# yumingj/Text2Human

Measured on AMD Instinct MI355X. Metric: 512x256 images/sec (sample_from_parsing), higher is better.
Workload: dtype f16 hi plane + e4m3 cross-term planes, f32 accumulate (hidden err 4e-5, tokens exact); exact-f32: exact_fp32_path

## Files before the change

### text2human_amd/csrc/attention.hip

```cpp
#include <stdlib.h>

#include <type_traits>

#include "common.h"

namespace {

constexpr int HD = 64;
constexpr int QB = 128;
constexpr int KT = 64;
constexpr int K_LD = 68;
constexpr int V_LD = 64;
constexpr int O_LD = 68;
constexpr int KV_TILE = KT * K_LD + KT * V_LD;

__global__ __launch_bounds__(512) void mha_kernel(const float* __restrict__ qkv,
                                                  float* __restrict__ y, int T, int C,
                                                  int n_head, uint16_t* __restrict__ y_split, int* ovf) {
  __shared__ __attribute__((aligned(16))) float smem[2 * KV_TILE];
  static_assert(2 * KV_TILE >= 4 * 32 * 64 + 4 * 32 * O_LD, "LDS reuse layout");

  const int tid = threadIdx.x, lane = tid & 63, wave = tid >> 6;
  const int l31 = lane & 31, hh = lane >> 5;
  const int qw = wave & 3, kh = wave >> 2;
  int qt, head, b;
  {
    const int nqt = T / QB, total = gridDim.x, id = blockIdx.x;
    const int xcd = id & 7, slot = id >> 3, q = total >> 3, r = total & 7;
    const int lin = (xcd < r ? xcd * (q + 1) : r * (q + 1) + (xcd - r) * q) + slot;
    qt = lin % nqt;
    const int hb = lin / nqt;
    head = hb % n_head;
    b = hb / n_head;
  }
  const int q0 = qt * QB + qw * 32;
  const int ld = 3 * C;
  const float* base = qkv + (int64_t)b * T * ld + head * HD;

  float qf[32];
  {
    const float* qp = base + (int64_t)(q0 + l31) * ld + 32 * hh;
#pragma unroll
    for (int s4 = 0; s4 < 8; ++s4) {
      const f32x4 v = *reinterpret_cast<const f32x4*>(qp + 4 * s4);
#pragma unroll
      for (int e = 0; e < 4; ++e) qf[4 * s4 + e] = v[e] * 0.125f;
    }
  }

  f32x16 o_acc[2];
#pragma unroll
  for (int dt = 0; dt < 2; ++dt)
#pragma unroll
    for (int r = 0; r < 16; ++r) o_acc[dt][r] = 0.f;
  float m_run = -INFINITY, l_run = 0.f;

  const int s_half = tid >> 8, s_t = tid & 255;
  const int s_col4 = s_t & 15, s_row0 = s_t >> 4;
  float* const Ks_st = smem + s_half * KV_TILE;
  float* const Vs_st = Ks_st + KT * K_LD;
  const int half_keys = T / 2;
  f32x4 kreg[4], vreg[4];
  auto load_kv = [&](int it) {
#pragma unroll
    for (int i = 0; i < 4; ++i) {
      const int key = s_half * half_keys + it * KT + s_row0 + 16 * i;
      const float* p = base + (int64_t)key * ld + s_col4 * 4;
      kreg[i] = *reinterpret_cast<const f32x4*>(p + C);
      vreg[i] = *reinterpret_cast<const f32x4*>(p + 2 * C);
    }
  };
  auto store_kv = [&]() {
#pragma unroll
    for (int i = 0; i < 4; ++i) {
      const int r = s_row0 + 16 * i;
      *reinterpret_cast<f32x4*>(Ks_st + r * K_LD + s_col4 * 4) = kreg[i];
      *reinterpret_cast<f32x4*>(Vs_st + r * V_LD + s_col4 * 4) = vreg[i];
    }
  };

  const float* const Ks = smem + kh * KV_TILE;
  const float* const Vs = Ks + KT * K_LD;
  const int nit = half_keys / KT;
  load_kv(0);
  for (int it = 0; it < nit; ++it) {
    __syncthreads();
    store_kv();
    __syncthreads();
    if (it + 1 < nit) load_kv(it + 1);

#pragma unroll
    for (int ks = 0; ks < 2; ++ks) {
      f32x16 st;
#pragma unroll
      for (int r = 0; r < 16; ++r) st[r] = 0.f;
      const float* kp = Ks + (ks * 32 + l31) * K_LD + 32 * hh;
#pragma unroll
      for (int j = 0; j < 8; ++j) {
        const f32x4 kf = *reinterpret_cast<const f32x4*>(kp + 4 * j);
#pragma unroll
        for (int e = 0; e < 4; ++e)
          st = __builtin_amdgcn_mfma_f32_32x32x2f32(kf[e], qf[4 * j + e], st, 0, 0, 0);
      }
      float mx = st[0];
#pragma unroll
      for (int r = 1; r < 16; ++r) mx = fmaxf(mx, st[r]);
      mx = fmaxf(mx, __shfl_xor(mx, 32, 64));
      const float m_new = fmaxf(m_run, mx);
      const float alpha = (m_run == -INFINITY) ? 0.f : fast_exp(m_run - m_new);
      float psum = 0.f;
#pragma unroll
      for (int r = 0; r < 16; ++r) {
        st[r] = fast_exp(st[r] - m_new);
        psum += st[r];
      }
      psum += __shfl_xor(psum, 32, 64);
      l_run = l_run * alpha + psum;
      m_run = m_new;
#pragma unroll
      for (int dt = 0; dt < 2; ++dt)
#pragma unroll
        for (int r = 0; r < 16; ++r) o_acc[dt][r] *= alpha;
#pragma unroll
      for (int s = 0; s < 16; ++s) {
        const int key = ks * 32 + (s & 3) + 8 * (s >> 2) + 4 * hh;
        const float* vp = Vs + key * V_LD + l31;
#pragma unroll
        for (int dt = 0; dt < 2; ++dt)
          o_acc[dt] = __builtin_amdgcn_mfma_f32_32x32x2f32(vp[32 * dt], st[s], o_acc[dt], 0, 0, 0);
      }
    }
  }

  __syncthreads();
  float* const Ox = smem;
  float* const Mx = smem + 4 * 32 * 64;
  float* const Lx = Mx + 4 * 64;
  if (kh == 1) {
#pragma unroll
    for (int dt = 0; dt < 2; ++dt)
#pragma unroll
      for (int r = 0; r < 16; ++r) Ox[(qw * 32 + dt * 16 + r) * 64 + lane] = o_acc[dt][r];
    Mx[qw * 64 + lane] = m_run;
    Lx[qw * 64 + lane] = l_run;
  }
  __syncthreads();
  float inv_l = 0.f;
  if (kh == 0) {
    const float m2 = Mx[qw * 64 + lane], l2 = Lx[qw * 64 + lane];
    const float m = fmaxf(m_run, m2);
    const float a1 = expf(m_run - m), a2 = expf(m2 - m);
#pragma unroll
    for (int dt = 0; dt < 2; ++dt)
#pragma unroll
      for (int r = 0; r < 16; ++r)
        o_acc[dt][r] = o_acc[dt][r] * a1 + Ox[(qw * 32 + dt * 16 + r) * 64 + lane] * a2;
    inv_l = 1.0f / (l_run * a1 + l2 * a2);
  }
  __syncthreads();
  float* Os = smem + 4 * 32 * 64 + qw * 32 * O_LD;
  if (kh == 0) {
#pragma unroll
    for (int dt = 0; dt < 2; ++dt)
#pragma unroll
      for (int r = 0; r < 16; ++r) {
        const int d = dt * 32 + (r & 3) + 8 * (r >> 2) + 4 * hh;
        Os[l31 * O_LD + d] = o_acc[dt][r] * inv_l;
      }
  }
  __syncthreads();
  if (kh == 0) {
    const int64_t grow = (int64_t)b * T + q0;
#pragma unroll
    for (int it = 0; it < 4; ++it) {
      const int row = it * 8 + (lane >> 3), c8 = (lane & 7) * 8;
      const f32x4 va = *reinterpret_cast<const f32x4*>(Os + row * O_LD + c8);
      const f32x4 vb = *reinterpret_cast<const f32x4*>(Os + row * O_LD + c8 + 4);
      if (y) {
        *reinterpret_cast<f32x4*>(y + (grow + row) * C + head * HD + c8) = va;
        *reinterpret_cast<f32x4*>(y + (grow + row) * C + head * HD + c8 + 4) = vb;
      }
      if (y_split) t2h_store_split8(y_split, grow + row, C, head * HD + c8, va, vb, ovf);
    }
  }
}


typedef t2h_f16x8 f16x8;
typedef unsigned int u32x4 __attribute__((ext_vector_type(4)));

template <int J>
__device__ __forceinline__ void split8(const f32x16& x, f16x8& hi, f16x8& lo) {
#pragma unroll
  for (int e = 0; e < 8; ++e) {
    _Float16 a, b;
    t2h_split2(x[8 * J + e], a, b);
    hi[e] = a;
    lo[e] = b;
  }
}

#ifndef T2H_MHA_PACKED
#define T2H_MHA_PACKED 0
#endif
#ifdef T2H_MHA_TIMING
__device__ long long* g_mha_timing = nullptr;
#define TM_NOW() clock64()
#else
#define TM_NOW() 0ll
#endif

__device__ __forceinline__ void half_barrier(int* ctr, int target, int lane) {
  asm volatile("s_waitcnt lgkmcnt(0)" ::: "memory");
  if (lane == 0) __hip_atomic_fetch_add(ctr, 1, __ATOMIC_RELAXED, __HIP_MEMORY_SCOPE_WORKGROUP);
  while (__hip_atomic_load(ctr, __ATOMIC_RELAXED, __HIP_MEMORY_SCOPE_WORKGROUP) < target) __builtin_amdgcn_s_sleep(1);
  asm volatile("" ::: "memory");
}

constexpr int DK_TILE = KT * 256;
constexpr int DV_TILE = 2 * HD * 128;
constexpr int DKV_TILE = DK_TILE + DV_TILE;

template <int KH>
__global__ __launch_bounds__(512) void mha_split_pipe_kernel(const uint16_t* __restrict__ qk, int ld_cols,
                                                        const uint16_t* __restrict__ vt, float* __restrict__ y,
                                                        uint16_t* __restrict__ y_split, int T, int C, int n_head,
                                                        int* ovf, float y_x8_scale) {
  constexpr int NQW = 8 / KH;
  constexpr int EPI_B = KH == 2 ? (4 * 32 * 64 + 4 * 32 * O_LD) * 4 : NQW * 32 * O_LD * 4;
  constexpr int SMEM_B = 2 * KH * DKV_TILE > EPI_B ? 2 * KH * DKV_TILE : EPI_B;
  __shared__ __attribute__((aligned(16))) char smem_raw[SMEM_B + 16];
  float* const smem = reinterpret_cast<float*>(smem_raw);
  int* const bar = reinterpret_cast<int*>(smem_raw + SMEM_B);

  const int tid = threadIdx.x, lane = tid & 63;
  const int wave = __builtin_amdgcn_readfirstlane(tid >> 6);
  const long long tm0 = TM_NOW();
#ifdef T2H_MHA_TIMING
  const long long rt0 = (long long)__builtin_amdgcn_s_memrealtime();
#endif
  long long tm_stage = 0, tm_comp = 0;
  if (tid < 2) bar[tid] = 0;
  __syncthreads();
  const int l31 = lane & 31, hh = lane >> 5;
  const int qw = KH == 2 ? (wave & 3) : wave, kh = KH == 2 ? (wave >> 2) : 0;
  int qt, head, b;
  {
    const int nqt = T / (32 * NQW), total = gridDim.x, id = blockIdx.x;
    const int xcd = id & 7, slot = id >> 3, q = total >> 3, r = total & 7;
    const int lin = (xcd < r ? xcd * (q + 1) : r * (q + 1) + (xcd - r) * q) + slot;
    qt = lin % nqt;
    const int hb = lin / nqt;
    head = hb % n_head;
    b = hb / n_head;
  }
  const int q0 = qt * (32 * NQW) + qw * 32;
  const int64_t row_b = (int64_t)(ld_cols / 32) * T2H_SPLIT_TILE_B;
  const char* const qk_b = reinterpret_cast<const char*>(qk) + (int64_t)b * T * row_b;
  const int q_tile0 = 2 * head, k_tile0 = C / 32 + 2 * head;

  f16x8 qf[4][2];
  {
    const char* qp = qk_b + (int64_t)(q0 + l31) * row_b + q_tile0 * T2H_SPLIT_TILE_B + hh * 16;
#pragma unroll
    for (int kk = 0; kk < 4; ++kk)
#pragma unroll
      for (int pl = 0; pl < 2; ++pl)
        qf[kk][pl] = *reinterpret_cast<const f16x8*>(qp + (kk >> 1) * T2H_SPLIT_TILE_B + pl * 64 + (kk & 1) * 32);
  }

  f32x16 o_acc[2], o_lo[2];
#pragma unroll
  for (int dt = 0; dt < 2; ++dt)
#pragma unroll
    for (int r = 0; r < 16; ++r) o_acc[dt][r] = o_lo[dt][r] = 0.f;
  float m_run = -INFINITY, l_run = 0.f;

  const int half_keys = T / KH;
  const int w4 = qw;
  constexpr int CPW = 16 / NQW;
  const char* const vt_b = reinterpret_cast<const char*>(vt) + ((int64_t)(b * n_head + head) * 2 * HD) * T * 2;
  const unsigned lds_half = (unsigned)(uintptr_t)smem_raw + kh * (2 * DKV_TILE);
  const char* const kbase = qk_b + (int64_t)(kh * half_keys) * row_b + k_tile0 * T2H_SPLIT_TILE_B;
  const char* const vbase = vt_b + (int64_t)(kh * half_keys) * 2;
  const unsigned k_rowoff = (unsigned)(4 * CPW * w4 + (lane >> 4)) * (unsigned)row_b;
  const unsigned k_b16 = (unsigned)((lane & 15) ^ (lane >> 4) ^ ((4 * CPW * w4) & 15)) * 16;
  const unsigned v_rowoff = (unsigned)(8 * CPW * w4 + (lane >> 3)) * (unsigned)(T * 2);
  const unsigned v_b16 = (unsigned)((lane & 7) ^ (lane >> 4) ^ ((4 * CPW * w4) & 7)) * 16;
  auto dma16 = [&](unsigned voff, const char* sbase, unsigned lds_dst) {
    unsigned keep;
#ifndef T2H_MHA_DMA_POLICY
#define T2H_MHA_DMA_POLICY ""
#endif
    asm volatile("s_mov_b32 %0, m0\n\ts_mov_b32 m0, %3\n\ts_nop 0\n\tglobal_load_lds_dwordx4 %1, %2" T2H_MHA_DMA_POLICY "\n\ts_mov_b32 m0, %0"
                 : "=&s"(keep)
                 : "v"(voff), "s"(sbase), "s"(lds_dst)
                 : "memory");
  };
  auto dma_k = [&](int it, int buf) {
    const char* const sb = kbase + (int64_t)it * KT * row_b;
    const unsigned dst = __builtin_amdgcn_readfirstlane(lds_half + buf * DKV_TILE + CPW * w4 * 1024);
#pragma unroll
    for (int i = 0; i < CPW; ++i) dma16(k_rowoff + (unsigned)(4 * i) * (unsigned)row_b + (k_b16 ^ (64u * i)), sb, dst + i * 1024);
  };
  auto dma_v = [&](int it, int buf) {
    const char* const sb = vbase + it * KT * 2;
    const unsigned dst = __builtin_amdgcn_readfirstlane(lds_half + buf * DKV_TILE + DK_TILE + CPW * w4 * 1024);
#pragma unroll
    for (int i = 0; i < CPW; ++i) dma16(v_rowoff + (unsigned)(8 * i) * (unsigned)(T * 2) + (v_b16 ^ (64u * (i & 1))), sb, dst + i * 1024);
  };
  auto dma_landed = [] { asm volatile("s_waitcnt vmcnt(0)" ::: "memory"); };

  const char* const Ks0 = smem_raw + kh * (2 * DKV_TILE);
  const int nit = half_keys / KT;
  const unsigned xk16 = (unsigned)(hh ^ (l31 & 15)) * 16, xv16 = (unsigned)(hh ^ ((l31 >> 1) & 7)) * 16;
  auto s_tile = [&](const char* Ks, f32x16 (&st)[2], f32x16 (&st_lo)[2]) {
#pragma unroll
    for (int ks = 0; ks < 2; ++ks)
#pragma unroll
      for (int r = 0; r < 16; ++r) st[ks][r] = st_lo[ks][r] = 0.f;
#pragma unroll
    for (int kk = 0; kk < 4; ++kk) {
      f16x8 kf[2][2];
#pragma unroll
      for (int ks = 0; ks < 2; ++ks)
#pragma unroll
        for (int pl = 0; pl < 2; ++pl)
          kf[ks][pl] = *reinterpret_cast<const f16x8*>(
              Ks + (ks * 32 + l31) * 256 + ((unsigned)(((kk >> 1) * 8 + pl * 4 + (kk & 1) * 2) * 16) ^ xk16));
      st_lo[0] = __builtin_amdgcn_mfma_f32_32x32x16_f16(kf[0][1], qf[kk][0], st_lo[0], 0, 0, 0);
      st_lo[1] = __builtin_amdgcn_mfma_f32_32x32x16_f16(kf[1][1], qf[kk][0], st_lo[1], 0, 0, 0);
      st[0] = __builtin_amdgcn_mfma_f32_32x32x16_f16(kf[0][0], qf[kk][0], st[0], 0, 0, 0);
      st_lo[0] = __builtin_amdgcn_mfma_f32_32x32x16_f16(kf[0][0], qf[kk][1], st_lo[0], 0, 0, 0);
      st_lo[1] = __builtin_amdgcn_mfma_f32_32x32x16_f16(kf[1][0], qf[kk][1], st_lo[1], 0, 0, 0);
      st[1] = __builtin_amdgcn_mfma_f32_32x32x16_f16(kf[1][0], qf[kk][0], st[1], 0, 0, 0);
    }
  };

  int bar_n = 0;
  const long long tm1 = TM_NOW();
#ifdef T2H_MHA_TIMING
  const long long rt1 = (long long)__builtin_amdgcn_s_memrealtime();
#endif
  if (KH == 2 && kh == 1) __builtin_amdgcn_s_setprio(1);
  constexpr float SC = 0.125f * 1.44269504088896340736f;
  f32x16 sc[2];
  {
    f32x16 st[2], st_lo[2];
    dma_k(0, 0);
    dma_v(0, 0);
    if (nit > 1) dma_k(1, 1);
    dma_landed();
    half_barrier(bar + kh, bar_n += NQW, lane);
    s_tile(Ks0, st, st_lo);
#pragma unroll
    for (int ks = 0; ks < 2; ++ks)
#pragma unroll
      for (int r = 0; r < 16; ++r) sc[ks][r] = fmaf(st_lo[ks][r], T2H_SPLIT_LO_INV, st[ks][r]);
    half_barrier(bar + kh, bar_n += NQW, lane);
  }
  auto iteration = [&](int it, auto next_c) {
    constexpr bool NEXT = decltype(next_c)::value;
    const long long tb = TM_NOW();
    const int buf = it & 1;
    const char* const Vs = Ks0 + buf * DKV_TILE + DK_TILE;
    if (it + 2 < nit) dma_k(it + 2, buf);
    if (it + 1 < nit) dma_v(it + 1, buf ^ 1);
    float mx = -INFINITY;
#pragma unroll
    for (int ks = 0; ks < 2; ++ks)
#pragma unroll
      for (int r = 0; r < 16; ++r) mx = fmaxf(mx, sc[ks][r]);
    mx = fmaxf(mx, __shfl_xor(mx, 32, 64)) * SC;
    const float m_new = fmaxf(m_run, mx);
    if (__any(m_new > m_run)) {
      const float alpha = (m_run == -INFINITY) ? 0.f : __builtin_amdgcn_exp2f(m_run - m_new);
      l_run *= alpha;
#pragma unroll
      for (int dt = 0; dt < 2; ++dt)
#pragma unroll
        for (int r = 0; r < 16; ++r) {
          o_acc[dt][r] *= alpha;
          o_lo[dt][r] *= alpha;
        }
      m_run = m_new;
    }
    f32x16 sn[2], sn_lo[2];
    if constexpr (NEXT) s_tile(Ks0 + (buf ^ 1) * DKV_TILE, sn, sn_lo);
    float psum = 0.f;
#if T2H_MHA_PACKED
    typedef float f32x2_ __attribute__((ext_vector_type(2)));
    const f32x2_ sc2 = {SC, SC}, nm2 = {-m_run, -m_run};
    f32x2_ ps2 = {0.f, 0.f};
#endif
#pragma unroll
    for (int ks = 0; ks < 2; ++ks) {
#if T2H_MHA_PACKED
#pragma unroll
      for (int r = 0; r < 16; r += 2) {
        f32x2_ a = {sc[ks][r], sc[ks][r + 1]};
        a = __builtin_elementwise_fma(a, sc2, nm2);
        a[0] = __builtin_amdgcn_exp2f(a[0]);
        a[1] = __builtin_amdgcn_exp2f(a[1]);
        sc[ks][r] = a[0];
        sc[ks][r + 1] = a[1];
        ps2 += a;
      }
#else
#pragma unroll
      for (int r = 0; r < 16; ++r) {
        sc[ks][r] = __builtin_amdgcn_exp2f(fmaf(sc[ks][r], SC, -m_run));
        psum += sc[ks][r];
      }
#endif
#pragma unroll
      for (int j = 0; j < 2; ++j) {
        f16x8 pf[2];
        if (j == 0) split8<0>(sc[ks], pf[0], pf[1]);
        else split8<1>(sc[ks], pf[0], pf[1]);
        f16x8 vf[2][2];
#pragma unroll
        for (int dt = 0; dt < 2; ++dt)
#pragma unroll
          for (int pl = 0; pl < 2; ++pl)
            vf[dt][pl] = *reinterpret_cast<const f16x8*>(Vs + (pl * HD + dt * 32 + l31) * 128 +
                                                          ((unsigned)((ks * 4 + j * 2) * 16) ^ xv16));
        o_lo[0] = __builtin_amdgcn_mfma_f32_32x32x16_f16(vf[0][1], pf[0], o_lo[0], 0, 0, 0);
        o_lo[1] = __builtin_amdgcn_mfma_f32_32x32x16_f16(vf[1][1], pf[0], o_lo[1], 0, 0, 0);
        o_acc[0] = __builtin_amdgcn_mfma_f32_32x32x16_f16(vf[0][0], pf[0], o_acc[0], 0, 0, 0);
        o_lo[0] = __builtin_amdgcn_mfma_f32_32x32x16_f16(vf[0][0], pf[1], o_lo[0], 0, 0, 0);
        o_lo[1] = __builtin_amdgcn_mfma_f32_32x32x16_f16(vf[1][0], pf[1], o_lo[1], 0, 0, 0);
        o_acc[1] = __builtin_amdgcn_mfma_f32_32x32x16_f16(vf[1][0], pf[0], o_acc[1], 0, 0, 0);
      }
    }
#if T2H_MHA_PACKED
    psum = ps2[0] + ps2[1];
#endif
    psum += __shfl_xor(psum, 32, 64);
    l_run += psum;
    if constexpr (NEXT) {
#pragma unroll
      for (int ks = 0; ks < 2; ++ks)
#pragma unroll
        for (int r = 0; r < 16; ++r) sc[ks][r] = fmaf(sn_lo[ks][r], T2H_SPLIT_LO_INV, sn[ks][r]);
    }
    const long long tc = TM_NOW();
    tm_comp += tc - tb;
    if constexpr (NEXT) {
      dma_landed();
      half_barrier(bar + kh, bar_n += NQW, lane);
    }
    tm_stage += TM_NOW() - tc;
  };
  for (int it = 0; it + 1 < nit; ++it) iteration(it, std::true_type{});
  iteration(nit - 1, std::false_type{});

#pragma unroll
  for (int dt = 0; dt < 2; ++dt)
#pragma unroll
    for (int r = 0; r < 16; ++r) o_acc[dt][r] = fmaf(o_lo[dt][r], T2H_SPLIT_LO_INV, o_acc[dt][r]);
  const long long tm2 = TM_NOW();
#ifdef T2H_MHA_TIMING
  const long long rt2 = (long long)__builtin_amdgcn_s_memrealtime();
#endif
  __syncthreads();
  if constexpr (KH == 2) {
  float* const Ox = smem;
  float* const Mx = smem + 4 * 32 * 64;
  float* const Lx = Mx + 4 * 64;
  if (kh == 1) {
#pragma unroll
    for (int dt = 0; dt < 2; ++dt)
#pragma unroll
      for (int r = 0; r < 16; ++r) Ox[(qw * 32 + dt * 16 + r) * 64 + lane] = o_acc[dt][r];
    Mx[qw * 64 + lane] = m_run;
    Lx[qw * 64 + lane] = l_run;
  }
  __syncthreads();
  float inv_l = 0.f;
  if (kh == 0) {
    const float m2 = Mx[qw * 64 + lane], l2 = Lx[qw * 64 + lane];
    const float m = fmaxf(m_run, m2);
    const float a1 = exp2f(m_run - m), a2 = exp2f(m2 - m);
#pragma unroll
    for (int dt = 0; dt < 2; ++dt)
#pragma unroll
      for (int r = 0; r < 16; ++r)
        o_acc[dt][r] = o_acc[dt][r] * a1 + Ox[(qw * 32 + dt * 16 + r) * 64 + lane] * a2;
    inv_l = 1.0f / (l_run * a1 + l2 * a2);
  }
  __syncthreads();
  float* Os = smem + 4 * 32 * 64 + qw * 32 * O_LD;
  if (kh == 0) {
#pragma unroll
    for (int dt = 0; dt < 2; ++dt)
#pragma unroll
      for (int r = 0; r < 16; ++r) {
        const int d = dt * 32 + (r & 3) + 8 * (r >> 2) + 4 * hh;
        Os[l31 * O_LD + d] = o_acc[dt][r] * inv_l;
      }
  }
  __syncthreads();
  {
    const int64_t grow = (int64_t)b * T + q0;
#pragma unroll
    for (int it2 = 0; it2 < 2; ++it2) {
      const int it = it2 + 2 * kh;
      const int row = it * 8 + (lane >> 3), c8 = (lane & 7) * 8;
      const f32x4 va = *reinterpret_cast<const f32x4*>(Os + row * O_LD + c8);
      const f32x4 vb = *reinterpret_cast<const f32x4*>(Os + row * O_LD + c8 + 4);
      if (y) {
        *reinterpret_cast<f32x4*>(y + (grow + row) * C + head * HD + c8) = va;
        *reinterpret_cast<f32x4*>(y + (grow + row) * C + head * HD + c8 + 4) = vb;
      }
      if (y_split) {
        if (y_x8_scale > 0.f) t2h_store_x8_8<1>(y_split, grow + row, C, head * HD + c8, va, vb, y_x8_scale, ovf);
        else t2h_store_split8(y_split, grow + row, C, head * HD + c8, va, vb, ovf);
      }
    }
  }
  } else {
    const float inv_l = 1.0f / l_run;
    float* const Os = smem + qw * 32 * O_LD;
#pragma unroll
    for (int dt = 0; dt < 2; ++dt)
#pragma unroll
      for (int r = 0; r < 16; ++r) {
        const int d = dt * 32 + (r & 3) + 8 * (r >> 2) + 4 * hh;
        Os[l31 * O_LD + d] = o_acc[dt][r] * inv_l;
      }
    asm volatile("s_waitcnt lgkmcnt(0)" ::: "memory");
    const int64_t grow = (int64_t)b * T + q0;
#pragma unroll
    for (int it = 0; it < 4; ++it) {
      const int row = it * 8 + (lane >> 3), c8 = (lane & 7) * 8;
      const f32x4 va = *reinterpret_cast<const f32x4*>(Os + row * O_LD + c8);
      const f32x4 vb = *reinterpret_cast<const f32x4*>(Os + row * O_LD + c8 + 4);
      if (y) {
        *reinterpret_cast<f32x4*>(y + (grow + row) * C + head * HD + c8) = va;
        *reinterpret_cast<f32x4*>(y + (grow + row) * C + head * HD + c8 + 4) = vb;
      }
      if (y_split) {
        if (y_x8_scale > 0.f) t2h_store_x8_8<1>(y_split, grow + row, C, head * HD + c8, va, vb, y_x8_scale, ovf);
        else t2h_store_split8(y_split, grow + row, C, head * HD + c8, va, vb, ovf);
      }
    }
  }
#ifdef T2H_MHA_TIMING
  if (g_mha_timing && blockIdx.x == 8 && lane == 0 && (wave == 0 || wave == 4)) {
    long long* o = g_mha_timing + (wave == 4 ? 8 : 0);
    const long long te = clock64();
    o[0] = te - tm0; o[1] = tm1 - tm0; o[2] = tm_stage; o[3] = tm_comp; o[4] = te - tm2; o[5] = tm2 - tm1;
    const long long rte = (long long)__builtin_amdgcn_s_memrealtime();
    o[6] = rte - rt0; o[7] = (rt1 - rt0) | ((rt2 - rt1) << 32);
  }
#endif
}

thread_local int g_force_mha_form = 0;

}

static int pick_mha_form(int32_t B, int32_t T, int32_t n_head) {
  const int64_t wg2 = (int64_t)(T / QB) * n_head * B, wg1 = T % 256 == 0 ? (int64_t)(T / 256) * n_head * B : 0;
  return (wg1 > 0 && ((wg1 + 255) / 256) * 5 < ((wg2 + 255) / 256) * 3) ? 1 : 2;
}

extern "C" int t2h_mha_split_form(int32_t B, int32_t T, int32_t n_head) {
  T2H_REQUIRE(B > 0 && n_head > 0 && T > 0 && T % QB == 0, "t2h_mha_split_form: bad arguments (B=%d T=%d)", B, T);
  return pick_mha_form(B, T, n_head);
}

extern "C" int t2h_mha_split_force_form(int form) {
  const int old = g_force_mha_form;
  g_force_mha_form = (form == 1 || form == 2) ? form : 0;
  return old;
}

extern "C" int t2h_mha_noncausal_f32(const float* qkv, float* y, int32_t B, int32_t T,
                                     int32_t n_head, void* stream) {
  T2H_REQUIRE(qkv && y, "t2h_mha_noncausal_f32: NULL pointer");
  T2H_REQUIRE(B > 0 && n_head > 0, "t2h_mha_noncausal_f32: empty problem");
  T2H_REQUIRE(T > 0 && T % QB == 0, "t2h_mha_noncausal_f32: T=%d must be a multiple of %d", T, QB);
  T2H_REQUIRE(t2h_aligned16(qkv) && t2h_aligned16(y), "t2h_mha_noncausal_f32: 16-byte alignment");
  const int C = n_head * HD;
  dim3 grid((T / QB) * n_head * B), block(512);
  hipLaunchKernelGGL(mha_kernel, grid, block, 0, static_cast<hipStream_t>(stream), qkv, y, T, C, n_head,
                     static_cast<uint16_t*>(nullptr), static_cast<int*>(nullptr));
  T2H_CHECK_LAUNCH("t2h_mha_noncausal_f32");
  return T2H_OK;
}

extern "C" int t2h_mha_noncausal_split_f32(const float* qkv, uint16_t* y_split, int32_t B, int32_t T,
                                           int32_t n_head, int32_t* overflow_flag, void* stream) {
  T2H_REQUIRE(qkv && y_split, "t2h_mha_noncausal_split_f32: NULL pointer");
  T2H_REQUIRE(B > 0 && n_head > 0, "t2h_mha_noncausal_split_f32: empty problem");
  T2H_REQUIRE(T > 0 && T % QB == 0, "t2h_mha_noncausal_split_f32: T=%d must be a multiple of %d", T, QB);
  T2H_REQUIRE(t2h_aligned16(qkv) && t2h_aligned16(y_split), "t2h_mha_noncausal_split_f32: 16-byte alignment");
  const int C = n_head * HD;
  dim3 grid((T / QB) * n_head * B), block(512);
  int* ovf = overflow_flag;
  T2H_REQUIRE(ovf != nullptr, "t2h_mha_noncausal_split_f32: overflow_flag is NULL");
  hipLaunchKernelGGL(mha_kernel, grid, block, 0, static_cast<hipStream_t>(stream), qkv,
                     static_cast<float*>(nullptr), T, C, n_head, y_split, ovf);
  T2H_CHECK_LAUNCH("t2h_mha_noncausal_split_f32");
  return T2H_OK;
}

static int mha_split_launch(const uint16_t* qk_split, int32_t ld_cols, const uint16_t* vt, float* y, uint16_t* y_split,
                            float y_x8_scale, int32_t B, int32_t T, int32_t n_head, int32_t* overflow_flag, void* stream) {
  T2H_REQUIRE(qk_split && vt && (y || y_split), "t2h_mha_split_f32: NULL pointer");
  T2H_REQUIRE(B > 0 && n_head > 0, "t2h_mha_split_f32: empty problem");
  T2H_REQUIRE(T > 0 && T % QB == 0, "t2h_mha_split_f32: T=%d must be a multiple of %d", T, QB);
  const int C = n_head * HD;
  T2H_REQUIRE(ld_cols % 32 == 0 && ld_cols >= 2 * C, "t2h_mha_split_f32: ld_cols=%d must hold q and k (%d columns)",
              ld_cols, 2 * C);
  T2H_REQUIRE(t2h_aligned16(qk_split) && t2h_aligned16(vt) && (!y || t2h_aligned16(y)) &&
                  (!y_split || t2h_aligned16(y_split)),
              "t2h_mha_split_f32: 16-byte alignment");
  dim3 block(512);
  int* ovf = overflow_flag;
  T2H_REQUIRE(ovf != nullptr || y_split == nullptr, "t2h_mha_split_f32: overflow_flag is NULL (needed with y_split)");
  const int64_t wg2 = (int64_t)(T / QB) * n_head * B, wg1 = T % 256 == 0 ? (int64_t)(T / 256) * n_head * B : 0;
  int form = g_force_mha_form;
  if (form == 0) form = pick_mha_form(B, T, n_head);
  T2H_REQUIRE(form == 2 || wg1 > 0, "t2h_mha_split_f32: the all-keys form needs T %% 256 == 0");
  if (form == 1)
    hipLaunchKernelGGL(mha_split_pipe_kernel<1>, dim3((unsigned)wg1), block, 0, static_cast<hipStream_t>(stream), qk_split,
                       ld_cols, vt, y, y_split, T, C, n_head, ovf, y_x8_scale);
  else
    hipLaunchKernelGGL(mha_split_pipe_kernel<2>, dim3((unsigned)wg2), block, 0, static_cast<hipStream_t>(stream), qk_split,
                       ld_cols, vt, y, y_split, T, C, n_head, ovf, y_x8_scale);
  T2H_CHECK_LAUNCH("t2h_mha_split_f32");
  return T2H_OK;
}

extern "C" int t2h_mha_split_f32(const uint16_t* qk_split, int32_t ld_cols, const uint16_t* vt, float* y,
                                 uint16_t* y_split, int32_t B, int32_t T, int32_t n_head, int32_t* overflow_flag,
                                 void* stream) {
  return mha_split_launch(qk_split, ld_cols, vt, y, y_split, 0.f, B, T, n_head, overflow_flag, stream);
}

extern "C" int t2h_mha_split_x8_f32(const uint16_t* qk_split, int32_t ld_cols, const uint16_t* vt, uint16_t* y_x8,
                                    float y_scale, int32_t B, int32_t T, int32_t n_head, int32_t* overflow_flag,
                                    void* stream) {
  T2H_REQUIRE(y_x8 != nullptr && y_scale > 0.f, "t2h_mha_split_x8_f32: y_x8 is NULL or y_scale <= 0");
  return mha_split_launch(qk_split, ld_cols, vt, nullptr, y_x8, y_scale, B, T, n_head, overflow_flag, stream);
}

#ifdef T2H_MHA_TIMING
extern "C" int t2h_debug_set_mha_timing_buffer(void* dev_ptr) {
  return (int)hipMemcpyToSymbol(HIP_SYMBOL(g_mha_timing), &dev_ptr, sizeof(void*));
}
#endif
```

Baseline: 11.74.

## Split attention KV-half merge across both wave halves with a single barrier

Reworks the KH==2 epilogue of the split-pipe MHA kernel. Each key-half wave now publishes the half of its output accumulator that its partner needs, plus its running max and sum, into its own K/V tile region. After one barrier, both halves merge and normalise their own 32 output columns and write them out. This replaces the previous three-barrier flow in which one half did the whole merge while the other half sat idle. It also drops the dedicated epilogue LDS requirement, so shared memory usage may shrink. Explicit non-contracted multiplies and adds, with an FMA pattern chosen per element, are used so the merge arithmetic keeps the rounding of the old code.

Measured after the change: 11.63. No clear change (-0.9%).

```diff
diff --git a/text2human_amd/csrc/attention.hip b/text2human_amd/csrc/attention.hip
--- a/text2human_amd/csrc/attention.hip
+++ b/text2human_amd/csrc/attention.hip
@@ -210,6 +210,15 @@
 #define TM_NOW() 0ll
 #endif
 
+__device__ __forceinline__ float mul_rn(float a, float b) {
+#pragma clang fp contract(off)
+  return a * b;
+}
+__device__ __forceinline__ float add_rn(float a, float b) {
+#pragma clang fp contract(off)
+  return a + b;
+}
+
 __device__ __forceinline__ void half_barrier(int* ctr, int target, int lane) {
   asm volatile("s_waitcnt lgkmcnt(0)" ::: "memory");
   if (lane == 0) __hip_atomic_fetch_add(ctr, 1, __ATOMIC_RELAXED, __HIP_MEMORY_SCOPE_WORKGROUP);
@@ -227,7 +236,7 @@
                                                         uint16_t* __restrict__ y_split, int T, int C, int n_head,
                                                         int* ovf, float y_x8_scale) {
   constexpr int NQW = 8 / KH;
-  constexpr int EPI_B = KH == 2 ? (4 * 32 * 64 + 4 * 32 * O_LD) * 4 : NQW * 32 * O_LD * 4;
+  constexpr int EPI_B = KH == 2 ? 0 : NQW * 32 * O_LD * 4;
   constexpr int SMEM_B = 2 * KH * DKV_TILE > EPI_B ? 2 * KH * DKV_TILE : EPI_B;
   __shared__ __attribute__((aligned(16))) char smem_raw[SMEM_B + 16];
   float* const smem = reinterpret_cast<float*>(smem_raw);
@@ -463,63 +472,71 @@
 #ifdef T2H_MHA_TIMING
   const long long rt2 = (long long)__builtin_amdgcn_s_memrealtime();
 #endif
+  if constexpr (KH == 2) {
+  constexpr int XO_B = 4 * 64 * 16, XML_B = 64 * 8, OS_LD = 36, OS_B = 32 * OS_LD * 4;
+  static_assert(4 * XO_B <= DK_TILE && 4 * (XML_B + OS_B) <= DKV_TILE, "the merge areas leave the key half's K tile buffers");
+  typedef float f32x2 __attribute__((ext_vector_type(2)));
+  char* const mine_b = smem_raw + kh * (2 * DKV_TILE);
+  char* const partner_b = smem_raw + (kh ^ 1) * (2 * DKV_TILE);
+  f32x4* const Xo = reinterpret_cast<f32x4*>(mine_b + qw * XO_B);
+  f32x2* const Xml = reinterpret_cast<f32x2*>(mine_b + DKV_TILE + qw * XML_B);
+  const f32x4* const Po = reinterpret_cast<const f32x4*>(partner_b + qw * XO_B);
+  const f32x2* const Pml = reinterpret_cast<const f32x2*>(partner_b + DKV_TILE + qw * XML_B);
+  float* const Os = reinterpret_cast<float*>(mine_b + DKV_TILE + 4 * XML_B + qw * OS_B);
+  auto publish = [&](const f32x16& o) {
+#pragma unroll
+    for (int g = 0; g < 4; ++g) Xo[g * 64 + lane] = f32x4{o[4 * g], o[4 * g + 1], o[4 * g + 2], o[4 * g + 3]};
+    Xml[lane] = f32x2{m_run, l_run};
+  };
+  if (kh == 0) publish(o_acc[1]);
+  else publish(o_acc[0]);
   __syncthreads();
-  if constexpr (KH == 2) {
-  float* const Ox = smem;
-  float* const Mx = smem + 4 * 32 * 64;
-  float* const Lx = Mx + 4 * 64;
-  if (kh == 1) {
-#pragma unroll
-    for (int dt = 0; dt < 2; ++dt)
-#pragma unroll
-      for (int r = 0; r < 16; ++r) Ox[(qw * 32 + dt * 16 + r) * 64 + lane] = o_acc[dt][r];
-    Mx[qw * 64 + lane] = m_run;
-    Lx[qw * 64 + lane] = l_run;
-  }
-  __syncthreads();
-  float inv_l = 0.f;
-  if (kh == 0) {
-    const float m2 = Mx[qw * 64 + lane], l2 = Lx[qw * 64 + lane];
-    const float m = fmaxf(m_run, m2);
-    const float a1 = exp2f(m_run - m), a2 = exp2f(m2 - m);
-#pragma unroll
-    for (int dt = 0; dt < 2; ++dt)
-#pragma unroll
-      for (int r = 0; r < 16; ++r)
-        o_acc[dt][r] = o_acc[dt][r] * a1 + Ox[(qw * 32 + dt * 16 + r) * 64 + lane] * a2;
-    inv_l = 1.0f / (l_run * a1 + l2 * a2);
-  }
-  __syncthreads();
-  float* Os = smem + 4 * 32 * 64 + qw * 32 * O_LD;
-  if (kh == 0) {
-#pragma unroll
-    for (int dt = 0; dt < 2; ++dt)
-#pragma unroll
-      for (int r = 0; r < 16; ++r) {
-        const int d = dt * 32 + (r & 3) + 8 * (r >> 2) + 4 * hh;
-        Os[l31 * O_LD + d] = o_acc[dt][r] * inv_l;
-      }
-  }
-  __syncthreads();
+  const f32x2 pml = Pml[lane];
+  const float m0 = kh == 0 ? m_run : pml[0], l0 = kh == 0 ? l_run : pml[1];
+  const float m1 = kh == 0 ? pml[0] : m_run, l1 = kh == 0 ? pml[1] : l_run;
+  const float m = fmaxf(m0, m1);
+  const float a1 = exp2f(m0 - m), a2 = exp2f(m1 - m);
+  const float inv_l = 1.0f / add_rn(mul_rn(l0, a1), mul_rn(l1, a2));
+  auto finish = [&](const f32x16& o, auto g0_c) {
+    constexpr bool G0 = decltype(g0_c)::value;
+    f32x4 p[4];
+#pragma unroll
+    for (int g = 0; g < 4; ++g) p[g] = Po[g * 64 + lane];
+#pragma unroll
+    for (int g = 0; g < 4; ++g) {
+      f32x4 v;
+#pragma unroll
+      for (int e = 0; e < 4; ++e) {
+        const float g0 = G0 ? o[4 * g + e] : p[g][e], g1 = G0 ? p[g][e] : o[4 * g + e];
+        const float t = mul_rn(g1, a2);
+        v[e] = (4 * g + e < 14 ? fmaf(g0, a1, t) : add_rn(mul_rn(g0, a1), t)) * inv_l;
+      }
+      *reinterpret_cast<f32x4*>(Os + l31 * OS_LD + 8 * g + 4 * hh) = v;
+    }
+  };
+  if (kh == 0) finish(o_acc[0], std::true_type{});
+  else finish(o_acc[1], std::false_type{});
+  asm volatile("s_waitcnt lgkmcnt(0)" ::: "memory");
   {
     const int64_t grow = (int64_t)b * T + q0;
-#pragma unroll
-    for (int it2 = 0; it2 < 2; ++it2) {
-      const int it = it2 + 2 * kh;
-      const int row = it * 8 + (lane >> 3), c8 = (lane & 7) * 8;
-      const f32x4 va = *reinterpret_cast<const f32x4*>(Os + row * O_LD + c8);
-      const f32x4 vb = *reinterpret_cast<const f32x4*>(Os + row * O_LD + c8 + 4);
+    const int col = head * HD + kh * 32 + (lane & 3) * 8;
+#pragma unroll
+    for (int it = 0; it < 2; ++it) {
+      const int row = it * 16 + (lane >> 2);
+      const f32x4 va = *reinterpret_cast<const f32x4*>(Os + row * OS_LD + (lane & 3) * 8);
+      const f32x4 vb = *reinterpret_cast<const f32x4*>(Os + row * OS_LD + (lane & 3) * 8 + 4);
       if (y) {
-        *reinterpret_cast<f32x4*>(y + (grow + row) * C + head * HD + c8) = va;
-        *reinterpret_cast<f32x4*>(y + (grow + row) * C + head * HD + c8 + 4) = vb;
+        *reinterpret_cast<f32x4*>(y + (grow + row) * C + col) = va;
+        *reinterpret_cast<f32x4*>(y + (grow + row) * C + col + 4) = vb;
       }
       if (y_split) {
-        if (y_x8_scale > 0.f) t2h_store_x8_8<1>(y_split, grow + row, C, head * HD + c8, va, vb, y_x8_scale, ovf);
-        else t2h_store_split8(y_split, grow + row, C, head * HD + c8, va, vb, ovf);
+        if (y_x8_scale > 0.f) t2h_store_x8_8<1>(y_split, grow + row, C, col, va, vb, y_x8_scale, ovf);
+        else t2h_store_split8(y_split, grow + row, C, col, va, vb, ovf);
       }
     }
   }
   } else {
+    __syncthreads();
     const float inv_l = 1.0f / l_run;
     float* const Os = smem + qw * 32 * O_LD;
 #pragma unroll
```
